# patflick/psac

Measured on AMD Instinct MI355X. Metric: MChars/s SA+LCP build; rank-pair radix-sort HBM GB/s vs peak, higher is better.
Workload: dtype u64

## Files before the change

### include/psacx.h

```cpp
#ifndef PSACX_H
#define PSACX_H

#include <stddef.h>
#include <stdint.h>

#ifdef __cplusplus
extern "C" {
#endif

typedef struct psacx_ctx psacx_ctx;

enum {
    PSACX_OK = 0,
    PSACX_EINVAL = -1,
    PSACX_ERANGE = -2,
    PSACX_ENOMEM = -3,
    PSACX_EHIP = -4,
    PSACX_EDEVICE = -5,
    PSACX_ENOGPU = -6
};

enum {
    PSACX_LCP = 1u,
    PSACX_NO_FAST = 2u,
// ... 19 lines not shown
    psacx_round rounds[PSACX_MAX_ROUNDS];
    double ms_total;
    double ms_alphabet, ms_kmer, ms_sort_hist, ms_sort_scatter, ms_rebucket, ms_isa_scatter,
           ms_gather, ms_compact, ms_rmq_build, ms_finalize;
    double ms_sort_scatter3, ms_sort_tilehist, ms_sort_scatter2;
    uint64_t scatter_launches[3];
    uint64_t scatter_records[3];
    uint64_t scatter_bytes[3];
    uint64_t hist_bytes;
    uint64_t workspace_bytes;
    uint64_t onew_passes;
    uint64_t heavy_rounds;
    uint64_t heavy_records;
    uint64_t light_records;
    uint64_t level_gathers;
    double ms_host[9];
    uint64_t locate_fetches[2];
    uint64_t rebucket_1w;
} psacx_stats;


#define PSACX_STREAM_DEFAULT ((void*)(intptr_t)-1)
int psacx_create(psacx_ctx** out, int device, void* stream);
void psacx_destroy(psacx_ctx* ctx);
const char* psacx_strerror(int code);
const char* psacx_last_hip_error(const psacx_ctx* ctx);
int psacx_trim(psacx_ctx* ctx);

enum {
    PSACX_OPT_RESET = 0, PSACX_OPT_FORCE_DIET, PSACX_OPT_DIET_CAP, PSACX_OPT_ONE_STAGE, PSACX_OPT_TIES_RADIX, PSACX_OPT_NO_ONE_WORD,
    PSACX_OPT_ONE_WORD_ALWAYS, PSACX_OPT_ONE_WORD_MIN, PSACX_OPT_WIDEN_LAST, PSACX_OPT_NO_DIGIT_BYTES, PSACX_OPT_NO_BUCKET_SORT,
    PSACX_OPT_ISA_UPDATE, PSACX_OPT_GATHER, PSACX_OPT_NO_HEAVY, PSACX_OPT_NO_WHOLE, PSACX_OPT_NO_LAZY_RANKS, PSACX_OPT_NO_EARLY_OUT,
    PSACX_OPT_NO_SPREAD_CURSORS, PSACX_OPT_LOCATE_SHAPE, PSACX_OPT_LOCATE_COUNT, PSACX_OPT_GENERIC_REBUCKET,
    PSACX_OPT_COUNT
};
int psacx_configure(psacx_ctx* ctx, int option, uint64_t value);
int psacx_configure_from_env(psacx_ctx* ctx);
const char* psacx_debug_env(const char* name);

int psacx_construct_u32(psacx_ctx* ctx, const uint8_t* text, uint64_t n, uint32_t k,
                        uint32_t flags, uint32_t* SA, uint32_t* ISA, uint32_t* LCP);
int psacx_construct_u64(psacx_ctx* ctx, const uint8_t* text, uint64_t n, uint32_t k,
                        uint32_t flags, uint64_t* SA, uint64_t* ISA, uint64_t* LCP);
int psacx_construct_dev_u32(psacx_ctx* ctx, const uint8_t* d_text, uint64_t n, uint32_t k,
                            uint32_t flags, uint32_t* d_SA, uint32_t* d_ISA, uint32_t* d_LCP);
int psacx_construct_dev_u64(psacx_ctx* ctx, const uint8_t* d_text, uint64_t n, uint32_t k,
                            uint32_t flags, uint64_t* d_SA, uint64_t* d_ISA, uint64_t* d_LCP);

int psacx_construct_lc_u32(psacx_ctx* ctx, const uint8_t* text, uint64_t n, uint32_t k, uint32_t flags,
                           uint32_t* SA, uint32_t* ISA, uint32_t* LCP, uint8_t* Lc);
int psacx_construct_lc_u64(psacx_ctx* ctx, const uint8_t* text, uint64_t n, uint32_t k, uint32_t flags,
                           uint64_t* SA, uint64_t* ISA, uint64_t* LCP, uint8_t* Lc);
int psacx_construct_lc_dev_u32(psacx_ctx* ctx, const uint8_t* d_text, uint64_t n, uint32_t k, uint32_t flags,
                               uint32_t* d_SA, uint32_t* d_ISA, uint32_t* d_LCP, uint8_t* d_Lc);
int psacx_construct_lc_dev_u64(psacx_ctx* ctx, const uint8_t* d_text, uint64_t n, uint32_t k, uint32_t flags,
                               uint64_t* d_SA, uint64_t* d_ISA, uint64_t* d_LCP, uint8_t* d_Lc);

int psacx_construct_gsa_u32(psacx_ctx* ctx, const uint8_t* text, uint64_t n, const uint64_t* offsets, uint64_t m,
                            uint32_t k, uint32_t flags, uint32_t* SA, uint32_t* ISA, uint32_t* LCP);
int psacx_construct_gsa_u64(psacx_ctx* ctx, const uint8_t* text, uint64_t n, const uint64_t* offsets, uint64_t m,
                            uint32_t k, uint32_t flags, uint64_t* SA, uint64_t* ISA, uint64_t* LCP);
int psacx_construct_gsa_dev_u32(psacx_ctx* ctx, const uint8_t* d_text, uint64_t n, const uint64_t* d_offsets, uint64_t m,
                                uint32_t k, uint32_t flags, uint32_t* d_SA, uint32_t* d_ISA, uint32_t* d_LCP);
int psacx_construct_gsa_dev_u64(psacx_ctx* ctx, const uint8_t* d_text, uint64_t n, const uint64_t* d_offsets, uint64_t m,
                                uint32_t k, uint32_t flags, uint64_t* d_SA, uint64_t* d_ISA, uint64_t* d_LCP);

// ... 243 lines not shown
```

### psac_amd/_lib.py

```python
import ctypes as C
import os

_HERE = os.path.dirname(os.path.abspath(__file__))
LIB_PATH = os.path.join(_HERE, "lib", "libpsacx.so")

PSACX_LCP = 1
PSACX_NO_FAST = 2
PSACX_PROFILE = 4
PSACX_MAX_ROUNDS = 72
PSACX_MATCH_SUFFIXES = 1

OPTIONS = {"reset": 0, "force_diet": 1, "diet_cap": 2, "one_stage": 3, "ties_radix": 4, "no_one_word": 5, "one_word_always": 6, "one_word_min": 7,
           "widen_last": 8, "no_digit_bytes": 9, "no_bucket_sort": 10, "isa_update": 11, "gather": 12, "no_heavy": 13, "no_whole": 14, "no_lazy_ranks": 15, "no_early_out": 16,
           "no_spread_cursors": 17, "locate_shape": 18, "locate_count": 19, "generic_rebucket": 20}
MULTI_OPTIONS = {"layout": 1, "slab": 2, "output_slack": 3, "trace": 4, "wire_piece": 5, "pieces": 6, "check_chunks": 7, "global_refine_sort": 8,
                 "one_stage": 9, "two_word": 10, "one_word": 11, "no_slices": 12, "slice_wide": 13, "slice_shape": 14}
MULTI_FORCE_WIRE, MULTI_NO_RCCL, MULTI_SHM = 1, 2, 4
ENV_KNOBS = bool(os.environ.get("PSACX_ENV_KNOBS"))
if ENV_KNOBS and os.environ.get("PSACX_LIB"):
    LIB_PATH = os.environ["PSACX_LIB"]

EXPORTS = [
    "psacx_create", "psacx_destroy", "psacx_strerror", "psacx_last_hip_error", "psacx_trim", "psacx_configure", "psacx_configure_from_env", "psacx_debug_env",
    "psacx_construct_u32", "psacx_construct_u64", "psacx_construct_dev_u32", "psacx_construct_dev_u64",
    "psacx_construct_gsa_u32", "psacx_construct_gsa_u64", "psacx_construct_gsa_dev_u32", "psacx_construct_gsa_dev_u64",
    "psacx_construct_lc_u32", "psacx_construct_lc_u64", "psacx_construct_lc_dev_u32", "psacx_construct_lc_dev_u64",
    "psacx_get_stats", "psacx_profile", "psacx_check_dev_u32", "psacx_check_dev_u64", "psacx_check_gsa_dev_u32", "psacx_check_gsa_dev_u64", "psacx_pair_sort_dev_u32", "psacx_pair_sort_dev_u64", "psacx_ansv_u32",
    "psacx_ansv_u64", "psacx_ansv_dev_u32", "psacx_ansv_dev_u64", "psacx_suffix_tree_u32", "psacx_suffix_tree_u64", "psacx_suffix_tree_dev_u32", "psacx_suffix_tree_dev_u64",
    "psacx_check_suffix_tree_dev_u32", "psacx_check_suffix_tree_dev_u64",
    "psacx_suffix_tree_gsa_u32", "psacx_suffix_tree_gsa_u64", "psacx_suffix_tree_gsa_dev_u32", "psacx_suffix_tree_gsa_dev_u64",
    "psacx_check_suffix_tree_gsa_dev_u32", "psacx_check_suffix_tree_gsa_dev_u64", "psacx_dev_alloc", "psacx_dev_free", "psacx_copy_h2d", "psacx_copy_d2h", "psacx_sync",
    "psacx_rand_dna", "psacx_synth_text_dev",
    "psacx_lookup_table_dev_u32", "psacx_lookup_table_dev_u64", "psacx_locate_dev_u32", "psacx_locate_dev_u64", "psacx_locate_u32", "psacx_locate_u64",
    "psacx_string_ends_dev", "psacx_lookup_table_gsa_dev_u32", "psacx_lookup_table_gsa_dev_u64", "psacx_locate_gsa_dev_u32", "psacx_locate_gsa_dev_u64",
    "psacx_locate_gsa_u32", "psacx_locate_gsa_u64", "psacx_occurrences_dev_u32", "psacx_occurrences_dev_u64",
    "psacx_match_dev_u32", "psacx_match_dev_u64", "psacx_match_gsa_dev_u32", "psacx_match_gsa_dev_u64",
    "psacx_match_u32", "psacx_match_u64", "psacx_match_gsa_u32", "psacx_match_gsa_u64",
    "psacx_rmq_index_dev_u32", "psacx_rmq_index_dev_u64", "psacx_rmq_dev_u32", "psacx_rmq_dev_u64", "psacx_lce_dev_u32", "psacx_lce_dev_u64",
    "psacx_rmq_u32", "psacx_rmq_u64", "psacx_lce_u32", "psacx_lce_u64",
    "psacx_multi_create", "psacx_multi_unique_id", "psacx_multi_create_rank", "psacx_multi_destroy", "psacx_multi_nranks",
    "psacx_multi_nlocal", "psacx_multi_uses_rccl", "psacx_multi_last_error", "psacx_multi_ctx", "psacx_multi_construct_dev_u32",
    "psacx_multi_construct_dev_u64", "psacx_multi_construct_u32", "psacx_multi_construct_u64", "psacx_multi_get_stats",
    "psacx_multi_check_dev_u32", "psacx_multi_check_dev_u64", "psacx_multi_check_gsa_dev_u32", "psacx_multi_check_gsa_dev_u64", "psacx_multi_ansv_dev_u32", "psacx_multi_ansv_dev_u64",
    "psacx_multi_construct_gsa_dev_u32", "psacx_multi_construct_gsa_dev_u64", "psacx_multi_construct_gsa_u32", "psacx_multi_construct_gsa_u64",
    "psacx_multi_suffix_tree_dev_u32", "psacx_multi_suffix_tree_dev_u64", "psacx_multi_suffix_tree_u32", "psacx_multi_suffix_tree_u64",
    "psacx_multi_left_chars_dev_u32", "psacx_multi_left_chars_dev_u64", "psacx_multi_construct_lc_u32", "psacx_multi_construct_lc_u64",
    "psacx_multi_configure", "psacx_multi_configure_from_env", "psacx_multi_create_ex", "psacx_multi_create_rank_ex", "psacx_multi_get_memory", "psacx_multi_transport", "psacx_multi_get_wire", "psacx_multi_get_phases", "psacx_multi_last_form",
# ... 169 lines not shown
```

### psac_amd/csrc/construct.hpp

```cpp
#pragma once
#include <chrono>
#include <thread>
#include "engine.hpp"
#include "bucket_sort.hpp"
#include "heavy_keys.hpp"

namespace psacx {

constexpr int SCAN_ITEMS = 8;
#ifndef RB1W_BLOCK
#define RB1W_BLOCK 512
#endif
template <typename T> struct ScanCfg {
    static constexpr int BLOCK = sizeof(T) == 8 ? 512 : 768;
    static constexpr int TILE = BLOCK * SCAN_ITEMS;
};
constexpr int SCAN_TILE_MIN = 512 * SCAN_ITEMS;

constexpr unsigned SCAN_CHUNKS = 4096, SCAN_CHUNK = 1024 * 4;
template <typename T> struct Work {
    T *bsa;
    SortBufs<T> x, y;
    SortBufs<T> ry;
    T *pos_a, *pos_b;
// ... 598 lines not shown
                                               keep ? &onew_view : nullptr, dig,
                                               (in1.k1 == w.x.k1 && onew_pad_total<T>(n)) ? ONEW_PAD : (uint64_t)0, tie_bytes);
                if (rc1 == PSACX_RETRY_1STAGE) {
                    two_stage = false; retry_one_stage = true; one_word = false;
                } else if (rc1 == PSACX_RETRY_1W) {
                    one_word = false;
                    PSACX_TRY(make_keys(hist_in_keys));
                }
                else {
                    PSACX_TRY(rc1);
                    sorted.k1 = reinterpret_cast<T*>(s1); sorted.k2 = nullptr; sorted.v = d_sa;
                    packed1 = true;
                    onew_recs = keep;
                }
            }
        } else one_word = false;
        if (retry_one_stage) continue;
        if (!one_word)
        PSACX_TRY(pair_sort<T>(c, w.sc, in1, alt1, n, true, bits_w1, 0, w.diet ? (T*)nullptr : d_sa, &sorted, r0,
                               ks.spec, n, true, lo1, hist_in_keys ? (int)lo1 : -1));
        if (w.diet && sorted.v != d_sa)
            PSACX_HIP(c, hipMemcpyAsync(d_sa, sorted.v, n * sizeof(T), hipMemcpyDeviceToDevice, c->stream));
        T* S1 = sorted.k1;
        T* const S2 = w.diet ? w.x.k2 : first_alt.k2;
        T* free_k1 = (S1 == w.x.k1) ? w.y.k1 : w.x.k1;
        constexpr int TB = 256, TI = sizeof(T) == 8 ? 32 : 16, TG = 8;
        unsigned long long* d_big = reinterpret_cast<unsigned long long*>(w.d_totals + 2);
        unsigned long long* h_big = reinterpret_cast<unsigned long long*>(c->pinned + 64);
        {
            ProfScope ps(c, TC_GATHER);
            PSACX_HIP(c, hipMemsetAsync(d_big, 0, sizeof(unsigned long long), c->stream));
            const uint64_t nb = (n + (uint64_t)TB * TI - 1) / ((uint64_t)TB * TI);
            if constexpr (sizeof(T) == 8) {
                if (onew_recs)
                    hipLaunchKernelGGL((tie_resolve_1w_kernel<TB, TI, TG>), dim3((unsigned)nb), dim3(TB), 0, c->stream, reinterpret_cast<uint64_t*>(S1),
                                       reinterpret_cast<uint64_t*>(free_k1), reinterpret_cast<uint64_t*>(S2), n, onew_view, d_text, n, tab, ks, d_big,
                                       (const uint8_t*)tie_bytes);
            }
            if (!kn.ties_radix && !onew_recs)
                hipLaunchKernelGGL((tie_resolve_kernel<T, TB, TI, TG>), dim3((unsigned)nb), dim3(TB), 0, c->stream, S1, d_sa, S2, n, lo1,
                                   d_text, n, tab, ks, d_big, packed1);
            PSACX_HIP(c, hipGetLastError());
        }
        PSACX_HIP(c, hipMemcpyAsync(h_big, d_big, sizeof(unsigned long long), hipMemcpyDeviceToHost, c->stream));
        PSACX_HIP(c, hipStreamSynchronize(c->stream));
        if constexpr (sizeof(T) == 8) {
            if (onew_recs && *h_big) {
                ProfScope ps(c, TC_GATHER);
                hipLaunchKernelGGL(onew_widen_kernel<0>, dim3(grid_for(c, n, 256, 8)), dim3(256), 0, c->stream, reinterpret_cast<const uint64_t*>(S1), n, onew_view,
                                   reinterpret_cast<uint64_t*>(free_k1), reinterpret_cast<uint64_t*>(d_sa));
                PSACX_HIP(c, hipGetLastError());
                std::swap(S1, free_k1);
                sorted.k1 = S1;
                onew_recs = false;
            }
        }
        if (*h_big || kn.ties_radix) {
            const uint64_t ntiles = (n + ScanCfg<T>::TILE - 1) / ScanCfg<T>::TILE;
            {
                ProfScope ps(c, TC_COMPACT);
                hipLaunchKernelGGL((count_active_kernel<T, ScanCfg<T>::BLOCK, SCAN_ITEMS>), dim3((unsigned)ntiles), dim3(ScanCfg<T>::BLOCK), 0,
                                   c->stream, S1, n, (T)0, (T)0, w.d_nact, lo1, w.d_nunf);
                PSACX_HIP(c, hipGetLastError());
            }
            SortBufs<T> a, b, s2;
            if (w.diet) { a = w.ry; b.k1 = w.bsa; b.k2 = w.x.v; b.v = free_k1; }
            else { a.k1 = free_k1; a.k2 = first_alt.v; a.v = first_in.v; b.k1 = w.bsa; b.k2 = w.pos_b; b.v = d_isa; }
// ... 642 lines not shown
```

### psac_amd/csrc/engine.hpp

```cpp
#pragma once
#include <hip/hip_runtime.h>

#include <algorithm>
#include <cstdio>
#include <cstdlib>
#include <cstring>
#include <condition_variable>
#include <functional>
#include <map>
#include <mutex>
#include <string>
#include <thread>
#include <sched.h>
#include <pthread.h>
#include <cctype>
#include <cstdio>
#include <vector>

#include "../../include/psacx.h"
#include "radix.hpp"
#include "sa_kernels.hpp"

namespace psacx {

enum TimerCat {
    TC_ALPHABET = 0, TC_KMER, TC_SORT_HIST, TC_SORT_SCATTER, TC_SORT_SCATTER3, TC_SORT_SCATTER2, TC_SORT_TILEHIST, TC_REBUCKET, TC_ISA_SCATTER,
    TC_GATHER, TC_COMPACT, TC_RMQ_BUILD, TC_FINALIZE, TC_TOTAL, TC_COUNT
};

}

namespace psacx { struct HostPool; }

namespace psacx {
struct Knobs {
    bool force_diet = false;
    uint64_t diet_cap = 0;
    bool one_stage = false;
    bool ties_radix = false;
    bool no_one_word = false;
    bool one_word_always = false;
    unsigned one_word_min = 24;
    int isa_update = 0;
    bool no_digit_bytes = false;
    bool no_bucket_sort = false;
    int gather = 0;
    bool no_heavy = false;
    bool no_early_out = false;
    bool no_lazy_ranks = false;
    bool no_whole = false;
    bool widen_last = false;
    bool no_spread_cursors = false;
    bool generic_rebucket = false;
    int locate_shape = 0;
    bool locate_count = false;
};

}

struct psacx_ctx {
    int device = 0;
    hipStream_t stream = nullptr;
    bool own_stream = false;
    char* slab = nullptr;
    size_t slab_bytes = 0;
    char* aux = nullptr;
    size_t aux_bytes = 0;
    char* pinned = nullptr;
    char* pinned_dev = nullptr;
    size_t pinned_bytes = 0;
    char* io = nullptr;
    size_t io_bytes = 0;
    static constexpr int STAGE_SLOTS = 4;
    char* stage[STAGE_SLOTS] = {nullptr, nullptr, nullptr, nullptr};
    char* dstage = nullptr;
    size_t stage_bytes = 0;
    hipEvent_t stage_ev[STAGE_SLOTS] = {nullptr, nullptr, nullptr, nullptr};
    hipStream_t copy_stream[2] = {nullptr, nullptr};
    hipEvent_t narrow_ev[STAGE_SLOTS] = {nullptr, nullptr, nullptr, nullptr};
    void (*first_round_hook)(void*) = nullptr;
    void* first_round_hook_arg = nullptr;
    hipStream_t early_stream = nullptr;
    hipEvent_t early_ev = nullptr;
    unsigned long long* early_word = nullptr;
    psacx::HostPool* hpool = nullptr;
    std::multimap<size_t, void*>* pool = nullptr;
// ... 880 lines not shown
    *s1 = cur;
    return PSACX_OK;
}
inline int prefix_sort_1w(psacx_ctx* c, SortScratch& sc, uint64_t* k0, uint64_t* a, uint64_t* sa_out, uint64_t n, unsigned lo1, unsigned lead,
                          psacx_round* rs, uint64_t** s1, const uint8_t* text, uint64_t n_text, const CodeTable& tab, const KeyShape& ks, bool probe,
                          OneWordView* view_out = nullptr, uint8_t* dig = nullptr, uint64_t pad = 0, uint8_t* tie_bytes = nullptr) {
    constexpr int BLOCK = 512, ITEMS = 8, TILE0 = BLOCK * ITEMS;
    constexpr int TILE = BLOCK * PSACX_1W_ITEMS;
    const unsigned low = lead - RADIX_BITS;
    const unsigned sfield = 64 - low;
    const uint64_t ntiles = (n + TILE0 - 1) / TILE0;
    char* const scratch = sc.d_desc;
    const unsigned slab0 = slab_tiles_for(ntiles);
    const uint64_t nslabs0 = (ntiles + slab0 - 1) / slab0;
    unsigned* tile_hist0 = reinterpret_cast<unsigned*>(scratch + 256);
    unsigned long long* slab_tot0 = reinterpret_cast<unsigned long long*>(scratch + 256 + ((ntiles * RADIX * sizeof(unsigned) + 255) & ~(size_t)255));
    unsigned long long* base0 = sc.d_base;
    {
        ProfScope ps(c, TC_KMER);
        const uint64_t stride = std::max<uint64_t>(64, n >> 20), samples = n / stride;
        uint64_t slots = 1; while (slots < 4 * samples) slots <<= 1;
        unsigned long long* table = reinterpret_cast<unsigned long long*>(scratch + 256);
        unsigned long long* d_dups = reinterpret_cast<unsigned long long*>(scratch + 128);
        if (256 + slots * 8 <= sc.desc_bytes && samples >= 1024 && probe) {
            PSACX_HIP(c, hipMemsetAsync(scratch, 0, 256 + slots * 8, c->stream));
            hipLaunchKernelGGL((prefix_dup_probe_kernel<uint64_t>), dim3((unsigned)((samples + 255) / 256)), dim3(256), 0, c->stream, text, n_text, tab, ks, lo1,
                               stride, samples, table, slots, d_dups);
            PSACX_HIP(c, hipGetLastError());
            PSACX_HIP(c, hipMemcpyAsync(sc.h_base, d_dups, sizeof(unsigned long long), hipMemcpyDeviceToHost, c->stream));
            PSACX_HIP(c, hipStreamSynchronize(c->stream));
            if (sc.h_base[0] * 4 >= samples * 3) return PSACX_RETRY_1STAGE;
            if (sc.h_base[0] * 8 > samples) return PSACX_RETRY_1W;
        }
        hipLaunchKernelGGL((top_digit_hist_kernel<uint64_t, BLOCK, ITEMS>), dim3((unsigned)ntiles), dim3(BLOCK), 0, c->stream, text, n, n_text, tab, ks, tile_hist0);
        PSACX_HIP(c, hipGetLastError());
    }
    {
        ProfScope ps(c, TC_SORT_TILEHIST);
        hipLaunchKernelGGL(radix_slab_scan_kernel<0>, dim3((unsigned)nslabs0), dim3(RADIX), 0, c->stream, tile_hist0, ntiles, slab_tot0, slab0);
        hipLaunchKernelGGL(radix_top_scan_kernel<0>, dim3(1), dim3(RADIX), 0, c->stream, slab_tot0, nslabs0, base0);
        PSACX_HIP(c, hipGetLastError());
    }
    PSACX_HIP(c, hipMemcpyAsync(sc.h_base, base0, RADIX * sizeof(unsigned long long), hipMemcpyDeviceToHost, c->stream));
    PSACX_HIP(c, hipStreamSynchronize(c->stream));
    unsigned long long* h_tabs = sc.h_base + RADIX;
    for (int d = 0; d < RADIX; ++d) h_tabs[d] = sc.h_base[d];
    h_tabs[RADIX] = n;
    const OneWordLayout lay = onew_layout<TILE>(h_tabs, ntiles);
    if (lay.need > sc.desc_bytes || lay.vtiles >= (1ull << 31)) return PSACX_RETRY_1W;
    {
        ProfScope ps(c, TC_KMER);
        PSACX_HIP(c, hipMemsetAsync(scratch, 0, 256, c->stream));
        hipLaunchKernelGGL((key_scatter1w_kernel<BLOCK, ITEMS>), dim3((unsigned)ntiles), dim3(BLOCK), 0, c->stream, text, n, n_text, tab, ks, pad ? k0 : a, (int)(lo1 + low),
                           base0, tile_hist0, slab_tot0, reinterpret_cast<unsigned*>(scratch), sort_chunk_for(n, true), slab0, lo1 | (sfield << 16), (uint64_t)0,
                           (uint8_t*)nullptr, 0, pad);
        PSACX_HIP(c, hipGetLastError());
    }
    uint64_t* cur = nullptr;
    if (pad) PSACX_TRY(onew_bucket_passes(c, scratch, h_tabs, lay, k0, a, sa_out, sfield, low, lo1, n, &cur, view_out, dig, pad, tie_bytes));
    else PSACX_TRY(onew_bucket_passes(c, scratch, h_tabs, lay, a, k0, sa_out, sfield, low, lo1, n, &cur, view_out, dig, 0, tie_bytes));
    *s1 = cur;
    if (rs) { rs->sort_passes = (uint32_t)((low + RADIX_BITS - 1) / RADIX_BITS + 1); rs->sort_passes_skipped = 0; }
    return PSACX_OK;
}

}
```

### psac_amd/csrc/psacx_abi.hip

```cpp
#include "engine.hpp"

namespace psacx {
int construct_dev_u32(psacx_ctx*, const uint8_t*, uint64_t, uint32_t, uint32_t, uint32_t*, uint32_t*, uint32_t*);
int construct_dev_u64(psacx_ctx*, const uint8_t*, uint64_t, uint32_t, uint32_t, uint64_t*, uint64_t*, uint64_t*);
int construct_host_u32(psacx_ctx*, const uint8_t*, uint64_t, uint32_t, uint32_t, uint32_t*, uint32_t*, uint32_t*);
int construct_gsa_host_u32(psacx_ctx*, const uint8_t*, uint64_t, const uint64_t*, uint64_t, uint32_t, uint32_t, uint32_t*, uint32_t*, uint32_t*);
int construct_gsa_dev_u32(psacx_ctx*, const uint8_t*, uint64_t, const uint64_t*, uint64_t, uint32_t, uint32_t, uint32_t*, uint32_t*, uint32_t*);
int construct_gsa_host_u64(psacx_ctx*, const uint8_t*, uint64_t, const uint64_t*, uint64_t, uint32_t, uint32_t, uint64_t*, uint64_t*, uint64_t*);
int construct_gsa_dev_u64(psacx_ctx*, const uint8_t*, uint64_t, const uint64_t*, uint64_t, uint32_t, uint32_t, uint64_t*, uint64_t*, uint64_t*);
int construct_lc_host_u32(psacx_ctx*, const uint8_t*, uint64_t, uint32_t, uint32_t, uint32_t*, uint32_t*, uint32_t*, uint8_t*);
int construct_lc_host_u64(psacx_ctx*, const uint8_t*, uint64_t, uint32_t, uint32_t, uint64_t*, uint64_t*, uint64_t*, uint8_t*);
int construct_lc_dev_u32(psacx_ctx*, const uint8_t*, uint64_t, uint32_t, uint32_t, uint32_t*, uint32_t*, uint32_t*, uint8_t*);
int construct_lc_dev_u64(psacx_ctx*, const uint8_t*, uint64_t, uint32_t, uint32_t, uint64_t*, uint64_t*, uint64_t*, uint8_t*);
int construct_host_u64(psacx_ctx*, const uint8_t*, uint64_t, uint32_t, uint32_t, uint64_t*, uint64_t*, uint64_t*);
int pair_sort_dev_u32(psacx_ctx*, uint32_t*, uint32_t*, uint32_t*, uint64_t, uint32_t);
int pair_sort_dev_u64(psacx_ctx*, uint64_t*, uint64_t*, uint64_t*, uint64_t, uint32_t);
int check_dev_u32(psacx_ctx*, const uint8_t*, uint64_t, const uint32_t*, const uint32_t*, const uint32_t*, uint64_t*);
int check_dev_u64(psacx_ctx*, const uint8_t*, uint64_t, const uint64_t*, const uint64_t*, const uint64_t*, uint64_t*);
int check_gsa_dev_u32(psacx_ctx*, const uint8_t*, uint64_t, const uint64_t*, uint64_t, const uint32_t*, const uint32_t*, const uint32_t*, uint64_t*);
int check_gsa_dev_u64(psacx_ctx*, const uint8_t*, uint64_t, const uint64_t*, uint64_t, const uint64_t*, const uint64_t*, const uint64_t*, uint64_t*);
int synth_text_dev(psacx_ctx*, uint8_t*, uint64_t, uint64_t, int, uint64_t, uint64_t);
int suffix_tree_host_u32(psacx_ctx*, const uint8_t*, uint64_t, const uint32_t*, const uint32_t*, uint64_t*, uint32_t*);
int suffix_tree_host_u64(psacx_ctx*, const uint8_t*, uint64_t, const uint64_t*, const uint64_t*, uint64_t*, uint32_t*);
int suffix_tree_dev_u32(psacx_ctx*, const uint8_t*, uint64_t, const uint32_t*, const uint32_t*, uint64_t*, uint32_t*, uint64_t*);
// ... 74 lines not shown
        case PSACX_EDEVICE: return "device-side failure (look-back timeout)";
        case PSACX_ENOGPU: return "no HIP device available";
        default: return "unknown error";
    }
}

const char* psacx_last_hip_error(const psacx_ctx* c) { return c ? c->hip_err.c_str() : ""; }

int psacx_configure(psacx_ctx* c, int option, uint64_t value) {
    if (!c) return PSACX_EINVAL;
    psacx::Knobs& k = c->knobs;
    switch (option) {
    case PSACX_OPT_RESET: k = psacx::Knobs(); return PSACX_OK;
    case PSACX_OPT_FORCE_DIET: k.force_diet = value != 0; return PSACX_OK;
    case PSACX_OPT_DIET_CAP: k.diet_cap = value; return PSACX_OK;
    case PSACX_OPT_ONE_STAGE: k.one_stage = value != 0; return PSACX_OK;
    case PSACX_OPT_TIES_RADIX: k.ties_radix = value != 0; return PSACX_OK;
    case PSACX_OPT_NO_ONE_WORD: k.no_one_word = value != 0; return PSACX_OK;
    case PSACX_OPT_ONE_WORD_ALWAYS: k.one_word_always = value != 0; return PSACX_OK;
    case PSACX_OPT_ONE_WORD_MIN: if (value > 62) return PSACX_EINVAL; k.one_word_min = value ? (unsigned)std::max<uint64_t>(16, value) : 24u; return PSACX_OK;
    case PSACX_OPT_WIDEN_LAST: k.widen_last = value != 0; return PSACX_OK;
    case PSACX_OPT_NO_DIGIT_BYTES: k.no_digit_bytes = value != 0; return PSACX_OK;
    case PSACX_OPT_NO_BUCKET_SORT: k.no_bucket_sort = value != 0; return PSACX_OK;
    case PSACX_OPT_ISA_UPDATE: if (value > 2) return PSACX_EINVAL; k.isa_update = (int)value; return PSACX_OK;
    case PSACX_OPT_GATHER: if (value > 2) return PSACX_EINVAL; k.gather = (int)value; return PSACX_OK;
    case PSACX_OPT_NO_HEAVY: k.no_heavy = value != 0; return PSACX_OK;
    case PSACX_OPT_NO_WHOLE: k.no_whole = value != 0; return PSACX_OK;
    case PSACX_OPT_NO_LAZY_RANKS: k.no_lazy_ranks = value != 0; return PSACX_OK;
    case PSACX_OPT_NO_EARLY_OUT: k.no_early_out = value != 0; return PSACX_OK;
    case PSACX_OPT_NO_SPREAD_CURSORS: k.no_spread_cursors = value != 0; return PSACX_OK;
    case PSACX_OPT_LOCATE_SHAPE: if (value > 2) return PSACX_EINVAL; k.locate_shape = (int)value; return PSACX_OK;
    case PSACX_OPT_LOCATE_COUNT: k.locate_count = value != 0; return PSACX_OK;
    case PSACX_OPT_GENERIC_REBUCKET: k.generic_rebucket = value != 0; return PSACX_OK;
    default: return PSACX_EINVAL;
    }
}

const char* psacx_debug_env(const char* name) { return name ? getenv(name) : nullptr; }

int psacx_configure_from_env(psacx_ctx* c) {
    if (!c) return PSACX_EINVAL;
    static const struct { const char* name; int option; } flags[] = {
        {"PSACX_FORCE_DIET", PSACX_OPT_FORCE_DIET}, {"PSACX_ONE_STAGE", PSACX_OPT_ONE_STAGE}, {"PSACX_TIES_RADIX", PSACX_OPT_TIES_RADIX},
        {"PSACX_NO_ONE_WORD", PSACX_OPT_NO_ONE_WORD}, {"PSACX_ONE_WORD_ALWAYS", PSACX_OPT_ONE_WORD_ALWAYS}, {"PSACX_WIDEN_LAST", PSACX_OPT_WIDEN_LAST},
        {"PSACX_NO_DIGIT_BYTES", PSACX_OPT_NO_DIGIT_BYTES}, {"PSACX_NO_BUCKET_SORT", PSACX_OPT_NO_BUCKET_SORT}, {"PSACX_NO_HEAVY", PSACX_OPT_NO_HEAVY},
        {"PSACX_NO_WHOLE", PSACX_OPT_NO_WHOLE}, {"PSACX_NO_LAZY_RANKS", PSACX_OPT_NO_LAZY_RANKS},
        {"PSACX_NO_EARLY_OUT", PSACX_OPT_NO_EARLY_OUT}, {"PSACX_NO_SPREAD_CURSORS", PSACX_OPT_NO_SPREAD_CURSORS},
        {"PSACX_LOCATE_COUNT", PSACX_OPT_LOCATE_COUNT}, {"PSACX_GENERIC_REBUCKET", PSACX_OPT_GENERIC_REBUCKET}};
    (void)psacx_configure(c, PSACX_OPT_RESET, 0);
    for (const auto& f : flags) if (psacx_debug_env(f.name)) (void)psacx_configure(c, f.option, 1);
    if (const char* e = psacx_debug_env("PSACX_DIET_CAP")) (void)psacx_configure(c, PSACX_OPT_DIET_CAP, strtoull(e, nullptr, 10));
    if (const char* e = psacx_debug_env("PSACX_ONE_WORD_MIN")) (void)psacx_configure(c, PSACX_OPT_ONE_WORD_MIN, strtoull(e, nullptr, 10));
    if (const char* e = psacx_debug_env("PSACX_ISA_UPDATE")) (void)psacx_configure(c, PSACX_OPT_ISA_UPDATE, e[0] == 's' ? 1 : 2);
    if (const char* e = psacx_debug_env("PSACX_LOCATE_SHAPE")) (void)psacx_configure(c, PSACX_OPT_LOCATE_SHAPE, e[0] == 'g' ? 2 : 1);
    if (const char* e = psacx_debug_env("PSACX_GATHER")) (void)psacx_configure(c, PSACX_OPT_GATHER, e[0] == 'f' ? 1 : 2);
    return PSACX_OK;
}

int psacx_trim(psacx_ctx* c) {
    if (!c) return PSACX_EINVAL;
    PSACX_HIP(c, hipSetDevice(c->device));
    PSACX_HIP(c, hipStreamSynchronize(c->stream));
    if (c->slab) { PSACX_HIP(c, hipFree(c->slab)); c->slab = nullptr; c->slab_bytes = 0; }
    if (c->aux) { PSACX_HIP(c, hipFree(c->aux)); c->aux = nullptr; c->aux_bytes = 0; }
    if (c->io) { PSACX_HIP(c, hipFree(c->io)); c->io = nullptr; c->io_bytes = 0; }
    if (c->dstage) { PSACX_HIP(c, hipFree(c->dstage)); c->dstage = nullptr; }
    for (int i = 0; i < psacx_ctx::STAGE_SLOTS; ++i) {
        if (c->stage[i]) { (void)hipHostFree(c->stage[i]); c->stage[i] = nullptr; }
        if (c->stage_ev[i]) { (void)hipEventDestroy(c->stage_ev[i]); c->stage_ev[i] = nullptr; }
    }
    delete c->hpool; c->hpool = nullptr;
    pool_flush(c);
    return PSACX_OK;
}

int psacx_construct_u32(psacx_ctx* c, const uint8_t* t, uint64_t n, uint32_t k, uint32_t f, uint32_t* sa, uint32_t* isa, uint32_t* lcp) {
    return construct_host_u32(c, t, n, k, f, sa, isa, lcp);
}
int psacx_construct_u64(psacx_ctx* c, const uint8_t* t, uint64_t n, uint32_t k, uint32_t f, uint64_t* sa, uint64_t* isa, uint64_t* lcp) {
    return construct_host_u64(c, t, n, k, f, sa, isa, lcp);
}
// ... 157 lines not shown
```

### psac_amd/csrc/sa_kernels.hpp

```cpp
#pragma once
#ifndef RB_WAVES_ATTR
#define RB_WAVES_ATTR
#endif
#ifndef RB_ABLATE
#define RB_ABLATE 0
#endif
#include <type_traits>
#include "dev_common.hpp"
#include "rebucket_1w_math.hpp"

namespace psacx {

constexpr int RADIX_P = 256;

struct CodeTable { uint16_t c[256]; };

template <typename T>
__device__ __forceinline__ void key_summary_add(unsigned long long* partials, T or1, T and1, T or2, T and2) {
    __shared__ unsigned long long red[4][16];
    or1 = wave_reduce<T>(or1, OpOr()); and1 = wave_reduce<T>(and1, OpAnd());
    or2 = wave_reduce<T>(or2, OpOr()); and2 = wave_reduce<T>(and2, OpAnd());
    const unsigned wave = threadIdx.x / WAVE, nw = (blockDim.x + WAVE - 1) / WAVE;
    const unsigned long long hi = ~(unsigned long long)(T)~(T)0;
    if (lane_id() == 0) {
// ... 210 lines not shown
    unsigned dig[ITEMS];
    const uint64_t i0 = rec0 - ks.spec;
    if (rec0 >= ks.spec && rec0 + ITEMS <= n && (i0 & ~7ull) + 24 <= n_text && (reinterpret_cast<uintptr_t>(text) & 7u) == 0) {
        const uint64_t* __restrict__ tw = reinterpret_cast<const uint64_t*>(text + (i0 & ~7ull));
        const uint64_t w0 = tw[0], w1 = tw[1], w2 = tw[2];
        const unsigned sh8 = (unsigned)(i0 & 7ull) * 8;
        const uint64_t lo = sh8 ? (w0 >> sh8) | (w1 << (64 - sh8)) : w0, hi = sh8 ? (w1 >> sh8) | (w2 << (64 - sh8)) : w1;
        const unsigned tmask = nch * lc >= 32 ? ~0u : ((1u << (nch * lc)) - 1u);
        unsigned t = 0;
        for (unsigned q = 0; q + 1 < nch; ++q) t = (t << lc) | (unsigned)ctab[(lo >> (8 * q)) & 255u];
#pragma unroll
        for (int j = 0; j < ITEMS; ++j) {
            const unsigned k = (unsigned)j + nch - 1;
            const unsigned ch = (unsigned)((k < 8 ? lo >> (8 * k) : hi >> (8 * (k - 8))) & 255u);
            t = ((t << lc) | (unsigned)ctab[ch]) & tmask;
            dig[j] = ((t >> down) << up) & 255u;
        }
    } else {
#pragma unroll 1
        for (int j = 0; j < ITEMS; ++j) {
            const uint64_t rec = rec0 + j;
            unsigned t = 0;
            if (rec < n) {
                const uint64_t i = record_suffix(rec, ks.spec, n);
                for (unsigned q = 0; q < nch; ++q) t = (t << lc) | (unsigned)((i + q < n_text) ? ctab[text[i + q]] : (uint16_t)0);
            }
            dig[j] = ((t >> down) << up) & 255u;
        }
    }
#pragma unroll
    for (int j = 0; j < ITEMS; ++j) if (rec0 + j < n) atomicAdd(&my[dig[j]], 1u);
    __syncthreads();
    for (int d = threadIdx.x; d < RADIX; d += BLOCK) tile_hist[(uint64_t)blockIdx.x * RADIX + d] = lh[0][d] + lh[1][d] + lh[2][d] + lh[3][d];
}

template <typename T>
__device__ __forceinline__ T packed_chars(const uint8_t* __restrict__ text, uint64_t n_text, const uint16_t* ctab, unsigned lc, uint64_t q0, unsigned cnt) {
    T w = 0;
    if (q0 + cnt + 32 <= n_text) {
        for (unsigned t0 = 0; t0 < cnt; t0 += 32) {
            uint64_t x[4];
#pragma unroll
            for (int c = 0; c < 4; ++c) { x[c] = 0; if (t0 + 8u * c < cnt) __builtin_memcpy(&x[c], text + q0 + t0 + 8u * c, 8); }
#pragma unroll
            for (int c = 0; c < 4; ++c) {
#pragma unroll
                for (int i = 0; i < 8; ++i)
                    if (t0 + 8u * c + i < cnt) w = (T)(w << lc) | (T)ctab[(unsigned)(x[c] >> (8 * i)) & 255u];
            }
        }
        return w;
    }
    for (unsigned t = 0; t < cnt; ++t) {
        const uint64_t q = q0 + t;
        w = (T)(w << lc) | (T)(q < n_text ? ctab[text[q]] : (uint16_t)0);
    }
    return w;
}
template <typename T>
__global__ void prefix_dup_probe_kernel(const uint8_t* __restrict__ text, uint64_t n_text, CodeTable tab, KeyShape ks, unsigned lo1, uint64_t stride,
                                        uint64_t samples, unsigned long long* __restrict__ table, uint64_t slots, unsigned long long* __restrict__ dups) {
    const uint64_t s = (uint64_t)blockIdx.x * blockDim.x + threadIdx.x;
    if (s >= samples) return;
    const uint64_t i = s * stride;
    const T w1 = packed_chars<T>(text, n_text, tab.c, ks.lc, i, ks.c1);
    const unsigned long long key = ((unsigned long long)w1 >> lo1) + 1ull;
// ... 1489 lines not shown
        const unsigned g = g0 + threadIdx.x / G;
        const bool live = g < ng;
        const uint64_t e = t0 + (live ? leaders[g] : 0u);
        const unsigned b = onew_bucket(ow, e);
        const uint64_t bend = ow.off[b + 1];
        const T rec = (live && e + m < bend) ? R[e + m] : (T)0;
        const T beyond = (live && e + G < bend) ? R[e + G] : (T)0;
        const T key = shfl<T>(rec >> ow.sfield, (int)seg0);
        const bool same = live && e + m < bend && (rec >> ow.sfield) == key;
        const unsigned mine = (unsigned)(__ballot(same) >> seg0) & ((1u << G) - 1u);
        const unsigned len = (unsigned)__builtin_ctz(~mine);
        const bool too_long = len == (unsigned)G && e + G < bend && (beyond >> ow.sfield) == key;
        const bool member = live && !too_long && m < len;
        if (live && too_long && m == 0) atomicAdd(big, 1ull);
        const T sa = rec & smask;
        T k1 = ~(T)0, k2 = ~(T)0;
        if (member) {
            window_low_and_word2<T>(text, n_text, ctab, ks, sa, (T)onew_word1(ow, b, rec), ow.lo1, k1, k2);
        }
        unsigned rank = 0;
#pragma unroll
        for (int j = 0; j < G; ++j) {
            const T o1 = shfl<T>(k1, (int)(seg0 + j)), o2 = shfl<T>(k2, (int)(seg0 + j));
            if (o1 < k1 || (o1 == k1 && (o2 < k2 || (o2 == k2 && (unsigned)j < m)))) ++rank;
        }
        const bool moved = ((unsigned)(__ballot(member && rank != m) >> seg0) & ((1u << G) - 1u)) != 0;
        if (member) {
            W1[e + rank] = k1; S2[e + rank] = k2;
            if (moved) R[e + rank] = (key << ow.sfield) | sa;
        }
    }
}

template <typename T, int BLOCK>
__global__ __launch_bounds__(BLOCK) void gather_prefix_ties_kernel(uint64_t cnt, T* __restrict__ K1, const T* __restrict__ V,
                                          const uint8_t* __restrict__ text, uint64_t n_text, CodeTable tab, KeyShape ks,
                                          T* __restrict__ K2, unsigned long long* __restrict__ summary, bool packed = false,
                                          const uint32_t* __restrict__ ord = nullptr, unsigned lo1 = 0, int v32 = 0) {
    __shared__ uint16_t ctab[256];
    for (int i = threadIdx.x; i < 256; i += BLOCK) ctab[i] = tab.c[i];
    __syncthreads();
    const uint64_t stride = (uint64_t)gridDim.x * blockDim.x;
    const T lowmask = lo1 ? (T)(((T)1 << lo1) - 1) : (T)0;
    T o1 = 0, a1 = ~(T)0, o2 = 0, a2 = ~(T)0;
    for (uint64_t j = (uint64_t)blockIdx.x * blockDim.x + threadIdx.x; j < cnt; j += stride) {
        T k1 = K1[j], k2;
        const uint64_t sa = v32 ? (uint64_t)reinterpret_cast<const uint32_t*>(V)[j] : (uint64_t)V[j];
        if (packed && ord) window_low_and_word2<T>(text, n_text, ctab, ks, sa, k1, lo1, k1, k2);
        else {
            k2 = window_word2<T>(text, n_text, ctab, ks, sa);
            if (packed) k1 = window_word1<T>(text, n_text, ctab, ks, sa);
        }
        if (ord) k1 = (T)(((T)ord[j] << lo1) | (k1 & lowmask));
        if (packed || ord) K1[j] = k1;
        K2[j] = k2;
        o1 |= k1; a1 &= k1; o2 |= k2; a2 &= k2;
    }
    key_summary_add<T>(summary, o1, a1, o2, a2);
}

template <typename T>
__global__ void scatter_prefix_ties_kernel(const T* __restrict__ pos, uint64_t cnt, const T* __restrict__ K1s,
                                           const T* __restrict__ K2s, const T* __restrict__ Vs, T* __restrict__ S1,
                                           T* __restrict__ S2, T* __restrict__ SA, unsigned merge_lo = 0) {
    const uint64_t stride = (uint64_t)gridDim.x * blockDim.x;
    const T lowmask = merge_lo ? (T)(((T)1 << merge_lo) - 1) : ~(T)0;
// ... 530 lines not shown
```

Baseline: 26450.

## Add wave-persistent kernels for top-digit histogram and one-word tie resolution

Result: faster. 26880, median of 6 (+1.6%).

```diff
diff --git a/include/psacx.h b/include/psacx.h
--- a/include/psacx.h
+++ b/include/psacx.h
@@ -75,6 +75,7 @@
     PSACX_OPT_ONE_WORD_ALWAYS, PSACX_OPT_ONE_WORD_MIN, PSACX_OPT_WIDEN_LAST, PSACX_OPT_NO_DIGIT_BYTES, PSACX_OPT_NO_BUCKET_SORT,
     PSACX_OPT_ISA_UPDATE, PSACX_OPT_GATHER, PSACX_OPT_NO_HEAVY, PSACX_OPT_NO_WHOLE, PSACX_OPT_NO_LAZY_RANKS, PSACX_OPT_NO_EARLY_OUT,
     PSACX_OPT_NO_SPREAD_CURSORS, PSACX_OPT_LOCATE_SHAPE, PSACX_OPT_LOCATE_COUNT, PSACX_OPT_GENERIC_REBUCKET,
+    PSACX_OPT_PLAIN_SIDE_KERNELS,
     PSACX_OPT_COUNT
 };
 int psacx_configure(psacx_ctx* ctx, int option, uint64_t value);
diff --git a/psac_amd/_lib.py b/psac_amd/_lib.py
--- a/psac_amd/_lib.py
+++ b/psac_amd/_lib.py
@@ -12,7 +12,8 @@
 
 OPTIONS = {"reset": 0, "force_diet": 1, "diet_cap": 2, "one_stage": 3, "ties_radix": 4, "no_one_word": 5, "one_word_always": 6, "one_word_min": 7,
            "widen_last": 8, "no_digit_bytes": 9, "no_bucket_sort": 10, "isa_update": 11, "gather": 12, "no_heavy": 13, "no_whole": 14, "no_lazy_ranks": 15, "no_early_out": 16,
-           "no_spread_cursors": 17, "locate_shape": 18, "locate_count": 19, "generic_rebucket": 20}
+           "no_spread_cursors": 17, "locate_shape": 18, "locate_count": 19, "generic_rebucket": 20,
+           "plain_side_kernels": 21}
 MULTI_OPTIONS = {"layout": 1, "slab": 2, "output_slack": 3, "trace": 4, "wire_piece": 5, "pieces": 6, "check_chunks": 7, "global_refine_sort": 8,
                  "one_stage": 9, "two_word": 10, "one_word": 11, "no_slices": 12, "slice_wide": 13, "slice_shape": 14}
 MULTI_FORCE_WIRE, MULTI_NO_RCCL, MULTI_SHM = 1, 2, 4
diff --git a/psac_amd/csrc/construct.hpp b/psac_amd/csrc/construct.hpp
--- a/psac_amd/csrc/construct.hpp
+++ b/psac_amd/csrc/construct.hpp
@@ -654,7 +654,12 @@
             PSACX_HIP(c, hipMemsetAsync(d_big, 0, sizeof(unsigned long long), c->stream));
             const uint64_t nb = (n + (uint64_t)TB * TI - 1) / ((uint64_t)TB * TI);
             if constexpr (sizeof(T) == 8) {
-                if (onew_recs)
+                const uint64_t nwt = (n + (uint64_t)WAVE * TI - 1) / ((uint64_t)WAVE * TI);
+                if (onew_recs && tie_bytes && !kn.plain_side_kernels)
+                    hipLaunchKernelGGL((tie_resolve_1w_waves_kernel<TB, TI, TG>), dim3((unsigned)grid_for(c, nwt * WAVE, TB, 4)), dim3(TB), 0, c->stream,
+                                       reinterpret_cast<uint64_t*>(S1), reinterpret_cast<uint64_t*>(free_k1), reinterpret_cast<uint64_t*>(S2), n, onew_view, d_text, n,
+                                       tab, ks, d_big, (const uint8_t*)tie_bytes, nwt);
+                else if (onew_recs)
                     hipLaunchKernelGGL((tie_resolve_1w_kernel<TB, TI, TG>), dim3((unsigned)nb), dim3(TB), 0, c->stream, reinterpret_cast<uint64_t*>(S1),
                                        reinterpret_cast<uint64_t*>(free_k1), reinterpret_cast<uint64_t*>(S2), n, onew_view, d_text, n, tab, ks, d_big,
                                        (const uint8_t*)tie_bytes);
diff --git a/psac_amd/csrc/engine.hpp b/psac_amd/csrc/engine.hpp
--- a/psac_amd/csrc/engine.hpp
+++ b/psac_amd/csrc/engine.hpp
@@ -52,6 +52,7 @@
     bool widen_last = false;
     bool no_spread_cursors = false;
     bool generic_rebucket = false;
+    bool plain_side_kernels = false;
     int locate_shape = 0;
     bool locate_count = false;
 };
@@ -998,7 +999,12 @@
             if (sc.h_base[0] * 4 >= samples * 3) return PSACX_RETRY_1STAGE;
             if (sc.h_base[0] * 8 > samples) return PSACX_RETRY_1W;
         }
-        hipLaunchKernelGGL((top_digit_hist_kernel<uint64_t, BLOCK, ITEMS>), dim3((unsigned)ntiles), dim3(BLOCK), 0, c->stream, text, n, n_text, tab, ks, tile_hist0);
+        static_assert(TILE0 == 64 * WAVE, "top_digit_hist_waves_kernel: a wave takes a tile of 64 records per lane");
+        if (c->knobs.plain_side_kernels || (reinterpret_cast<uintptr_t>(tile_hist0) & 15u))
+            hipLaunchKernelGGL((top_digit_hist_kernel<uint64_t, BLOCK, ITEMS>), dim3((unsigned)ntiles), dim3(BLOCK), 0, c->stream, text, n, n_text, tab, ks, tile_hist0);
+        else
+            hipLaunchKernelGGL((top_digit_hist_waves_kernel<256>), dim3((unsigned)grid_for(c, ntiles * WAVE, 256, 5)), dim3(256), 0, c->stream, text, n, n_text, tab, ks,
+                               ntiles, tile_hist0);
         PSACX_HIP(c, hipGetLastError());
     }
     {
diff --git a/psac_amd/csrc/psacx_abi.hip b/psac_amd/csrc/psacx_abi.hip
--- a/psac_amd/csrc/psacx_abi.hip
+++ b/psac_amd/csrc/psacx_abi.hip
@@ -130,6 +130,7 @@
     case PSACX_OPT_LOCATE_SHAPE: if (value > 2) return PSACX_EINVAL; k.locate_shape = (int)value; return PSACX_OK;
     case PSACX_OPT_LOCATE_COUNT: k.locate_count = value != 0; return PSACX_OK;
     case PSACX_OPT_GENERIC_REBUCKET: k.generic_rebucket = value != 0; return PSACX_OK;
+    case PSACX_OPT_PLAIN_SIDE_KERNELS: k.plain_side_kernels = value != 0; return PSACX_OK;
     default: return PSACX_EINVAL;
     }
 }
@@ -144,7 +145,8 @@
         {"PSACX_NO_DIGIT_BYTES", PSACX_OPT_NO_DIGIT_BYTES}, {"PSACX_NO_BUCKET_SORT", PSACX_OPT_NO_BUCKET_SORT}, {"PSACX_NO_HEAVY", PSACX_OPT_NO_HEAVY},
         {"PSACX_NO_WHOLE", PSACX_OPT_NO_WHOLE}, {"PSACX_NO_LAZY_RANKS", PSACX_OPT_NO_LAZY_RANKS},
         {"PSACX_NO_EARLY_OUT", PSACX_OPT_NO_EARLY_OUT}, {"PSACX_NO_SPREAD_CURSORS", PSACX_OPT_NO_SPREAD_CURSORS},
-        {"PSACX_LOCATE_COUNT", PSACX_OPT_LOCATE_COUNT}, {"PSACX_GENERIC_REBUCKET", PSACX_OPT_GENERIC_REBUCKET}};
+        {"PSACX_LOCATE_COUNT", PSACX_OPT_LOCATE_COUNT}, {"PSACX_GENERIC_REBUCKET", PSACX_OPT_GENERIC_REBUCKET},
+        {"PSACX_PLAIN_SIDE_KERNELS", PSACX_OPT_PLAIN_SIDE_KERNELS}};
     (void)psacx_configure(c, PSACX_OPT_RESET, 0);
     for (const auto& f : flags) if (psacx_debug_env(f.name)) (void)psacx_configure(c, f.option, 1);
     if (const char* e = psacx_debug_env("PSACX_DIET_CAP")) (void)psacx_configure(c, PSACX_OPT_DIET_CAP, strtoull(e, nullptr, 10));
diff --git a/psac_amd/csrc/sa_kernels.hpp b/psac_amd/csrc/sa_kernels.hpp
--- a/psac_amd/csrc/sa_kernels.hpp
+++ b/psac_amd/csrc/sa_kernels.hpp
@@ -266,6 +266,97 @@
     for (int j = 0; j < ITEMS; ++j) if (rec0 + j < n) atomicAdd(&my[dig[j]], 1u);
     __syncthreads();
     for (int d = threadIdx.x; d < RADIX; d += BLOCK) tile_hist[(uint64_t)blockIdx.x * RADIX + d] = lh[0][d] + lh[1][d] + lh[2][d] + lh[3][d];
+}
+
+template <int BLOCK>
+__global__ __launch_bounds__(BLOCK, 4) void top_digit_hist_waves_kernel(const uint8_t* __restrict__ text, uint64_t n, uint64_t n_text, CodeTable tab, KeyShape ks,
+                                                                        uint64_t ntiles, unsigned* __restrict__ tile_hist) {
+    constexpr int NW = BLOCK / WAVE, PER = 64, TILE = WAVE * PER, NP = 6, ND = 4 * NP;
+    static_assert(RADIX == 4 * WAVE, "a lane stores four counters");
+    __shared__ uint16_t ctab[256];
+    __shared__ __attribute__((aligned(16))) unsigned lh[NW][RADIX];
+    const unsigned wave = __builtin_amdgcn_readfirstlane(threadIdx.x / WAVE), lane = lane_id();
+    for (int i = threadIdx.x; i < 256; i += BLOCK) ctab[i] = tab.c[i];
+    for (int i = threadIdx.x; i < NW * RADIX; i += BLOCK) (&lh[0][0])[i] = 0;
+    __syncthreads();
+    unsigned* const my = lh[wave];
+    const unsigned lc = ks.lc;
+    const unsigned nch = (8 + lc - 1) / lc < ks.c1 ? (8 + lc - 1) / lc : ks.c1;
+    const unsigned down = nch * lc > 8 ? nch * lc - 8 : 0, up = nch * lc < 8 ? 8 - nch * lc : 0;
+    const unsigned tmask = (1u << (nch * lc)) - 1u;
+    const uint64_t nwaves = (uint64_t)gridDim.x * NW;
+    auto fetch = [&](uint64_t t, uint4 (&q)[NP], unsigned& lead) -> bool {
+        lead = 0;
+#pragma unroll
+        for (int i = 0; i < NP; ++i) q[i] = make_uint4(0, 0, 0, 0);
+        if (t >= ntiles) return false;
+        const uint64_t rec0 = t * TILE + (uint64_t)lane * PER;
+        if (rec0 < ks.spec || rec0 + PER > n) return false;
+        const uint64_t i0 = rec0 - ks.spec;
+        lead = (unsigned)(reinterpret_cast<uintptr_t>(text + i0) & 15u);
+        const unsigned np = (lead + PER + nch - 1 + 15) / 16;
+        if (i0 < lead || i0 - lead + 16ull * np > n_text) return false;
+        const uint4* __restrict__ a = reinterpret_cast<const uint4*>(text + (i0 - lead));
+#pragma unroll
+        for (int i = 0; i < NP; ++i) if ((unsigned)i < np) q[i] = a[i];
+        return true;
+    };
+    uint64_t tile = (uint64_t)blockIdx.x * NW + wave;
+    uint4 qa[NP];
+    unsigned la;
+    bool fa = fetch(tile, qa, la);
+    while (tile < ntiles) {
+        const uint64_t next = tile + nwaves;
+        uint4 qb[NP];
+        unsigned lb;
+        const bool fb = fetch(next, qb, lb);
+        if (fa) {
+            uint32_t w[ND + 1];
+#pragma unroll
+            for (int i = 0; i < NP; ++i) { w[4 * i] = qa[i].x; w[4 * i + 1] = qa[i].y; w[4 * i + 2] = qa[i].z; w[4 * i + 3] = qa[i].w; }
+            w[ND] = 0;
+            if (la) {
+#pragma unroll
+                for (int j = 0; j < ND; ++j) w[j] = __builtin_amdgcn_alignbyte(w[j + 1], w[j], la & 3u);
+                if (la & 4u) {
+#pragma unroll
+                    for (int j = 0; j + 1 < ND; ++j) w[j] = w[j + 1];
+                }
+                if (la & 8u) {
+#pragma unroll
+                    for (int j = 0; j + 2 < ND; ++j) w[j] = w[j + 2];
+                }
+            }
+            unsigned t = 0;
+#pragma unroll
+            for (int k = 0; k < PER + 7; ++k) {
+                if (k < PER || (unsigned)(k - PER + 1) < nch) {
+                    t = ((t << lc) | (unsigned)ctab[(w[k >> 2] >> (8 * (k & 3))) & 255u]) & tmask;
+                    if (k >= 7 || (unsigned)k + 1 >= nch) atomicAdd(&my[((t >> down) << up) & 255u], 1u);
+                }
+            }
+        } else {
+            const uint64_t rec0 = tile * TILE + (uint64_t)lane * PER;
+#pragma unroll 1
+            for (int j = 0; j < PER; ++j) {
+                const uint64_t rec = rec0 + j;
+                if (rec >= n) break;
+                const uint64_t i = record_suffix(rec, ks.spec, n);
+                unsigned t = 0;
+                for (unsigned q = 0; q < nch; ++q) t = (t << lc) | (unsigned)((i + q < n_text) ? ctab[text[i + q]] : (uint16_t)0);
+                atomicAdd(&my[((t >> down) << up) & 255u], 1u);
+            }
+        }
+        xrun_order();
+        uint4* const mine = reinterpret_cast<uint4*>(my) + lane;
+        const uint4 cnt = *mine;
+        *mine = make_uint4(0, 0, 0, 0);
+        reinterpret_cast<uint4*>(tile_hist + tile * RADIX)[lane] = cnt;
+        xrun_order();
+#pragma unroll
+        for (int i = 0; i < NP; ++i) qa[i] = qb[i];
+        la = lb; fa = fb; tile = next;
+    }
 }
 
 template <typename T>
@@ -1821,6 +1912,207 @@
     }
 }
 
+__device__ __forceinline__ void window_low_and_word2_wide(const uint8_t* __restrict__ text, uint64_t n_text, const uint16_t* ctab, const KeyShape& ks,
+                                                          uint64_t sa, uint64_t have, unsigned lo1, uint64_t& k1, uint64_t& k2) {
+    const unsigned lc = ks.lc;
+    const unsigned nlow = (lo1 + lc - 1) / lc < ks.c1 ? (lo1 + lc - 1) / lc : ks.c1;
+    const unsigned lowbits = nlow * lc;
+    const uint64_t q0 = sa + ks.c1 - nlow;
+    const unsigned L = nlow + ks.c2;
+    if (L > 64 || q0 + 64 > n_text) { window_low_and_word2<uint64_t>(text, n_text, ctab, ks, sa, have, lo1, k1, k2); return; }
+    uint32_t x[16];
+#pragma unroll
+    for (int c = 0; c < 8; ++c) {
+        uint64_t v = 0;
+        if ((unsigned)(8 * c) < L) __builtin_memcpy(&v, text + q0 + 8 * c, 8);
+        x[2 * c] = (uint32_t)v; x[2 * c + 1] = (uint32_t)(v >> 32);
+    }
+    uint64_t lo = 0, w2 = 0;
+#pragma unroll
+    for (int d = 0; d < 16; ++d) {
+        if ((unsigned)(4 * d) < L) {
+            const uint32_t e0 = ctab[x[d] & 255u], e1 = ctab[(x[d] >> 8) & 255u], e2 = ctab[(x[d] >> 16) & 255u], e3 = ctab[x[d] >> 24];
+            const uint32_t part = (((((e0 << lc) | e1) << lc) | e2) << lc) | e3;
+            const unsigned ab = L - 4u * d < 4u ? L - 4u * d : 4u;
+            const unsigned a = nlow > 4u * d ? (nlow - 4u * d < 4u ? nlow - 4u * d : 4u) : 0u;
+            const unsigned b = ab - a;
+            if (a == 4u) lo = (lo << (4u * lc)) | part;
+            else if (b == 4u) w2 = (w2 << (4u * lc)) | part;
+            else {
+                const uint64_t P = part;
+                if (a) lo = (lo << (a * lc)) | (P >> ((4u - a) * lc));
+                if (b) w2 = (w2 << (b * lc)) | ((P >> ((4u - ab) * lc)) & ((1ull << (b * lc)) - 1ull));
+            }
+        }
+    }
+    k1 = lowbits >= 64 ? lo : (((have >> lowbits) << lowbits) | lo);
+    k2 = w2;
+}
+
+template <int BLOCK, int ITEMS, int G>
+__global__ __launch_bounds__(BLOCK, 4) void tie_resolve_1w_waves_kernel(uint64_t* __restrict__ R, uint64_t* __restrict__ W1, uint64_t* __restrict__ S2,
+                                                                     uint64_t n, OneWordView ow, const uint8_t* __restrict__ text, uint64_t n_text,
+                                                                     CodeTable tab, KeyShape ks, unsigned long long* __restrict__ big,
+                                                                     const uint8_t* __restrict__ tb, uint64_t ntiles) {
+    typedef uint64_t T;
+    constexpr int NW = BLOCK / WAVE, WT = WAVE * ITEMS;
+    static_assert(ITEMS == 32, "a thread takes the 32 bytes of its places as two 16-byte pieces");
+    static_assert(G == 8, "eight lanes per group");
+    static_assert(WT < 65536, "pairs and places of a tile as 16-bit entries");
+    __shared__ uint16_t ctab[256];
+    __shared__ unsigned long long s_off[257];
+    __shared__ uint16_t cands[NW][WT + 2];
+    __shared__ uint16_t leaders[NW][WT / 2 + 2];
+    for (int i = threadIdx.x; i < 256; i += BLOCK) ctab[i] = tab.c[i];
+    for (int i = threadIdx.x; i < 257; i += BLOCK) s_off[i] = ow.off[i];
+    __syncthreads();
+    ow.off = s_off;
+    const unsigned wave = __builtin_amdgcn_readfirstlane(threadIdx.x / WAVE), lane = lane_id(), m = lane & (G - 1), seg0 = lane & ~(unsigned)(G - 1);
+    uint16_t* const cl = cands[wave];
+    uint16_t* const ll = leaders[wave];
+    const T smask = (1ull << ow.sfield) - 1;
+    auto starts_bucket = [&](uint64_t e) -> bool { return ow.off[onew_bucket(ow, e)] == e; };
+    auto fetch = [&](uint64_t tile, uint4& q0, uint4& q1, unsigned& ext) {
+        q0 = make_uint4(0, 0, 0, 0); q1 = q0; ext = 256u;
+        if (tile >= ntiles) return;
+        const uint64_t t0 = tile * WT, e0 = t0 + (uint64_t)lane * ITEMS;
+        if (e0 < n) { q0 = *reinterpret_cast<const uint4*>(tb + e0); q1 = *reinterpret_cast<const uint4*>(tb + e0 + 16); }
+        if (lane == 0 && t0) ext = tb[t0 - 1];
+        if (lane == WAVE - 1 && t0 + WT < n) ext = tb[t0 + WT];
+    };
+    struct GroupRecs { uint64_t e, bend; unsigned b; bool live; T rec; };
+    struct TileBucket { bool one; unsigned b; uint64_t end; };
+    auto tile_bucket = [&](uint64_t wb) -> TileBucket {
+        TileBucket t;
+        t.b = (unsigned)__builtin_amdgcn_readfirstlane((int)onew_bucket(ow, wb ? wb - 1 : 0));
+        t.end = ow.off[t.b + 1];
+        t.one = __builtin_amdgcn_readfirstlane((int)(t.end > wb + WT + G)) != 0;
+        return t;
+    };
+    auto load_groups = [&](uint64_t wb, const TileBucket& tk, unsigned g0, unsigned nl) -> GroupRecs {
+        GroupRecs r;
+        const unsigned g = g0 + lane / G;
+        r.live = g < nl;
+        r.e = wb + (r.live ? (unsigned)ll[g] : 0u);
+        r.b = tk.b; r.bend = tk.end;
+        if (!tk.one) { r.b = onew_bucket(ow, r.e); r.bend = ow.off[r.b + 1]; }
+        r.rec = (r.live && r.e + m < r.bend) ? R[r.e + m] : (T)0;
+        return r;
+    };
+    auto order_groups = [&](uint64_t wb, const TileBucket& tk, unsigned nl) {
+        if (nl == 0) return;
+        GroupRecs nx = load_groups(wb, tk, 0, nl);
+        for (unsigned g0 = 0; g0 < nl; g0 += WAVE / G) {
+            const GroupRecs c = nx;
+            if (g0 + WAVE / G < nl) nx = load_groups(wb, tk, g0 + WAVE / G, nl);
+            const T key = shfl<T>(c.rec >> ow.sfield, (int)seg0);
+            const bool same = c.live && c.e + m < c.bend && (c.rec >> ow.sfield) == key;
+            const unsigned mine = (unsigned)(__ballot(same) >> seg0) & ((1u << G) - 1u);
+            const unsigned len = (unsigned)__builtin_ctz(~mine);
+            const bool full = c.live && len == (unsigned)G && c.e + G < c.bend;
+            bool too_long = false;
+            if (__ballot(full)) too_long = full && (R[c.e + G] >> ow.sfield) == key;
+            const bool member = c.live && !too_long && m < len;
+            if (c.live && too_long && m == 0) atomicAdd(big, 1ull);
+            const T sa = c.rec & smask;
+            T k1 = ~(T)0, k2 = ~(T)0;
+            if (member) {
+                window_low_and_word2_wide(text, n_text, ctab, ks, sa, (T)onew_word1(ow, c.b, c.rec), ow.lo1, k1, k2);
+            }
+            unsigned rank = 0;
+#pragma unroll
+            for (int j = 0; j < G; ++j) {
+                const T o1 = shfl<T>(k1, (int)(seg0 + j)), o2 = shfl<T>(k2, (int)(seg0 + j));
+                if (o1 < k1 || (o1 == k1 && (o2 < k2 || (o2 == k2 && (unsigned)j < m)))) ++rank;
+            }
+            const bool moved = ((unsigned)(__ballot(member && rank != m) >> seg0) & ((1u << G) - 1u)) != 0;
+            if (member) {
+                W1[c.e + rank] = k1; S2[c.e + rank] = k2;
+                if (moved) R[c.e + rank] = (key << ow.sfield) | sa;
+            }
+        }
+    };
+    const uint64_t nwaves = (uint64_t)gridDim.x * NW;
+    uint64_t tile = (uint64_t)blockIdx.x * NW + wave;
+    uint4 a0, a1;
+    unsigned ax;
+    fetch(tile, a0, a1, ax);
+    uint64_t pwb = 0;
+    TileBucket ptk = {true, 0u, 0ull};
+    unsigned pnl = 0;
+    while (tile < ntiles) {
+        const uint64_t next = tile + nwaves;
+        uint4 b0, b1;
+        unsigned bx;
+        fetch(next, b0, b1, bx);
+        const unsigned long long any_big = __hip_atomic_load(big, __ATOMIC_RELAXED, __HIP_MEMORY_SCOPE_AGENT);
+        const uint64_t wb = tile * WT, e0 = wb + (uint64_t)lane * ITEMS;
+        const uint32_t w[8] = {a0.x, a0.y, a0.z, a0.w, a1.x, a1.y, a1.z, a1.w};
+        const unsigned first = w[0] & 255u, last = w[7] >> 24;
+        unsigned before = shfl<unsigned>(last, (int)((lane + WAVE - 1) & (WAVE - 1))), after = shfl<unsigned>(first, (int)((lane + 1) & (WAVE - 1)));
+        if (lane == 0) before = ax;
+        if (lane == WAVE - 1) after = ax;
+        uint64_t cand = 0;
+        {
+            unsigned prevb = before & 255u;
+#pragma unroll
+            for (int d = 0; d < 8; ++d) {
+                const uint32_t x = w[d] ^ ((w[d] << 8) | prevb);
+#pragma unroll
+                for (int k = 0; k < 4; ++k) if (((x >> (8 * k)) & 255u) == 0) cand |= 1ull << (4 * d + k);
+                prevb = w[d] >> 24;
+            }
+            if (before > 255u) cand &= ~1ull;
+            if (lane == WAVE - 1 && after == last) cand |= 1ull << ITEMS;
+            const uint64_t room = e0 < n ? n - e0 : 0;
+            if (room <= (uint64_t)ITEMS) cand &= (1ull << room) - 1ull;
+        }
+        const unsigned cnt = (unsigned)__builtin_popcountll(cand);
+        const unsigned incl = wave_scan_inclusive<unsigned>(cnt, OpSum());
+        const unsigned nc = (unsigned)__builtin_amdgcn_readlane((int)incl, WAVE - 1);
+        if (nc) {
+            unsigned o = incl - cnt;
+            while (cand) {
+                cl[o++] = (uint16_t)(lane * ITEMS + (unsigned)__builtin_ctzll(cand));
+                cand &= cand - 1;
+            }
+            xrun_order();
+        }
+        const unsigned p0 = lane < nc ? (unsigned)cl[lane] : ~0u;
+        T x0 = 0, y0 = 0;
+        if (lane < nc) { x0 = R[wb + p0 - 1]; y0 = R[wb + p0]; }
+        order_groups(pwb, ptk, any_big ? 0u : pnl);
+        xrun_order();
+        const TileBucket tk = tile_bucket(wb);
+        unsigned nl = 0;
+        {
+            unsigned carry_p = ~0u, carry_t = 0;
+            for (unsigned i0 = 0; i0 < nc; i0 += WAVE) {
+                const bool have = i0 + lane < nc;
+                unsigned p = p0;
+                T x = x0, y = y0;
+                if (i0) {
+                    p = have ? (unsigned)cl[i0 + lane] : ~0u;
+                    if (have) { x = R[wb + p - 1]; y = R[wb + p]; }
+                }
+                const unsigned tied = (have && (x >> ow.sfield) == (y >> ow.sfield) && (tk.one || !starts_bucket(wb + p))) ? 1u : 0u;
+                unsigned pp = shfl<unsigned>(p, (int)((lane + WAVE - 1) & (WAVE - 1))), pt = shfl<unsigned>(tied, (int)((lane + WAVE - 1) & (WAVE - 1)));
+                if (lane == 0) { pp = carry_p; pt = carry_t; }
+                const bool lead = tied && p != 0 && !(pt && pp + 1 == p);
+                const uint64_t L = __ballot(lead);
+                if (lead) ll[nl + (unsigned)__builtin_popcountll(L & lanemask_lt())] = (uint16_t)(p - 1);
+                nl += (unsigned)__builtin_popcountll(L);
+                carry_p = (unsigned)__builtin_amdgcn_readlane((int)p, WAVE - 1); carry_t = (unsigned)__builtin_amdgcn_readlane((int)tied, WAVE - 1);
+            }
+        }
+        xrun_order();
+        pwb = wb; ptk = tk; pnl = nl;
+        a0 = b0; a1 = b1; ax = bx;
+        tile = next;
+    }
+    order_groups(pwb, ptk, __hip_atomic_load(big, __ATOMIC_RELAXED, __HIP_MEMORY_SCOPE_AGENT) ? 0u : pnl);
+}
+
 template <typename T, int BLOCK>
 __global__ __launch_bounds__(BLOCK) void gather_prefix_ties_kernel(uint64_t cnt, T* __restrict__ K1, const T* __restrict__ V,
                                           const uint8_t* __restrict__ text, uint64_t n_text, CodeTable tab, KeyShape ks,
```
